# Amandaynzhou/CGC-Net

Measured on AMD Instinct MI355X. Metric: cell-graphs/sec (fwd+bwd), batch=32, ~1800 nodes/16 feat, higher is better.
Workload: dtype f32; 1 GPU; C3: full CGC-Net (3 conv blocks + 2 DiffPool) fwd+bwd+Adam, 32 graphs/GPU/step, ~1803 nodes, ~16159 edges/graph, 16 feat, max_num_nodes=11404 (C1=1140, C2=114), flags=shipped; global_batch=32, nodes_per_batch=57711, parallelism=dp1, includes=CSR build + fwd + loss + bwd + grad all-reduce + Adam, step_sequencer=True, node_order=draw order, fused_adam=True, optimiser=cgc_adam_step (one launch; torch fused Adam arithmetic)

## Files before the change

cgc-net_amd/_abi.py:

```python
import ctypes as C

P, I, F, D, L = C.c_void_p, C.c_int, C.c_float, C.c_double, C.c_int64

ABI_VERSION = 28

PROTOTYPES = {
    'cgc_abi_version': [],
    'cgc_csr_bad_edges_offset': [L, I, I],
    'cgc_csr_build': [P, L, I, I, P, P, P, P, P, P, P, P],
    'cgc_collate': [P, I, I, P, P, P, I, P, P, L, P, P],
    'cgc_farthest_point_sample': [P, P, I, I, P, P, P, P],
    'cgc_farthest_point_sample_table16': [P, P, I, I, P, P, P, P],
    'cgc_radius_knn_ws_ints': [I, I],
    'cgc_radius_knn': [P, P, I, I, F, I, I, P, P, P, P, P],
    'cgc_knn_emit_edges': [P, P, I, I, L, P, P],
    'cgc_nuclei_lds_max_pixels': [],
    'cgc_nuclei_ws_bytes': [I],
    'cgc_nuclei_label_pass': [P, I, I, I, I, P, P, P, P],
    'cgc_nuclei_big_ws_bytes': [I, L],
    'cgc_nuclei_features': [P, P, I, I, I, I, P, P, I, I, L, P, P, P, P, P],
    'cgc_bgr_to_gray': [P, L, P, P],
    'cgc_label_ws_bytes': [I, I, I],
    'cgc_label_components': [P, I, I, I, I, I, I, P, P, P, P],
    'cgc_label_sizes': [P, I, I, I, P, P],
# ... 74 lines not shown
    'cgc_region_outline_count': [P, P, I, I, I, I, I, P, P, P, P],
    'cgc_region_outline_cracks': [P, P, I, I, I, I, I, P, P, L, P, P, P],
    'cgc_region_outline_loops': [L, P, P, P, P, P],
    'cgc_region_outline_keys': [L, L, P, P, P, P, P, P],
    'cgc_region_outline_tables': [L, L, P, P, P, P, P, P, P, P, P],
    'cgc_region_outline_scatter': [L, L, I, P, P, P, P, P, P, P, P, P, P],
    'cgc_region_outline_compact': [L, L, P, P, P, P, P],
    'cgc_edge_renorm': [P, P, I, F, P, P],
    'cgc_csr_transpose_vals': [P, P, P, I, P, P],
    'cgc_csr_invdeg': [P, P, I, P, P],
    'cgc_graph_build': [P, L, I, F, P, P, P, P, P, P, P, P, P, P, P],
    'cgc_graph_build_local': [P, L, I, P, P, I, I, I, F, P, P, P, P, P, P, P, P, P, P, P],
    'cgc_graph_local_max_nodes': [],
    'cgc_spmm': [P, P, P, P, P, P, P, P, I, I, P],
    'cgc_spmm_graphs': [P, P, P, P, P, P, P, P, I, I, I, P, I, I, I, P, P],
    'cgc_gemm_f32': [I, I, I, I, I, F, P, I, P, I, F, P, I, P, I, L, L, L, P, I, I, I, P, P, P, P, P, P, P, P, L, I, P],
    'cgc_gemm_ws_floats': [],
    'cgc_gemm_split_count': [],
    'cgc_gemm_half_count': [],
    'cgc_gemm_half_ws_floats': [],
    'cgc_gemm_half_min_work': [L],
    'cgc_gemm_tuning': [I],
    'cgc_reduce_batch_sum': [P, P, I, L, F, P],
    'cgc_reduce_batched': [P, P, I, I, I, F, P],
    'cgc_stats_blocks': [I, I],
    'cgc_stats_ws_floats': [I, I],
    'cgc_l2norm_act_stats': [P, I, I, I, I, P, P, P, P, P],
    'cgc_bn_finalize': [P, I, D, F, F, P, P, P, P, P],
    'cgc_l2norm_act_bn': [P, I, I, I, I, P, P, P, D, F, F, P, P, P, P, P, P],
    'cgc_sage_wide_fwd': [P, I, P, P, I, I, I, I, I, P, I, P, I, P, D, F, F, P, P, P, P, P, P],
    'cgc_bn_running_stats': [P, P, I, F, P, P, P],
    'cgc_bn_act_apply': [P, I, I, I, P, P, P, P, P, I, P, I, P],
    'cgc_bn_bwd_reduce': [P, I, P, I, I, I, P, P, P, P, P],
    'cgc_bn_act_l2_bwd': [P, I, P, P, I, I, I, I, I, P, P, P, P, D, P, P, P, P],
    'cgc_sage_narrow_fwd': [P, I, P, P, I, I, I, I, I, P, P, I, P, D, F, F, P, P, P, P, P, P],
    'cgc_sage_narrow_ws_floats': [I, I, I],
    'cgc_sage_narrow_bwd': [P, I, P, P, I, I, I, I, I, P, P, P, P, D, P, I, I, P, P, I, P, P, P],
    'cgc_colsum': [P, I, I, I, P, P, P],
    'cgc_softmax_fwd': [P, I, I, I, P, P],
    'cgc_softmax_bwd': [P, P, I, I, I, P, P, P, P],
    'cgc_segment_max_fwd': [P, P, I, I, I, P, P, P],
    'cgc_segment_max_bwd': [P, P, I, I, P, P],
    'cgc_segment_max_bwd_full': [P, P, P, I, I, I, P, P],
    'cgc_jk_supported': [I],
    'cgc_jk_matrix_core': [I],
    'cgc_jk_lstm_fwd': [P, I, I, I, P, P, P, P, P, P, P],
    'cgc_jk_lstm_bwd': [P, P, I, I, I, P, P, P, P, P, P, P, P, P, P],
    'cgc_jk_bwd_ws_floats': [I],
    'cgc_jk_lstm_bwd_params': [P, P, I, I, I, P, P, P, P, P, P, P, P, P],
    'cgc_jk_lstm_bwd_flat': [P, P, I, I, I, P, P, P, P, P, P, P, P, P],
    'cgc_jk_param_grad_floats': [I],
    'cgc_jk_unpack_param_grads': [P, I, P, P],
# ... 46 lines not shown
```

cgc-net_amd/csrc/exec.hip:

```cpp
#include <stdio.h>
#include <stdlib.h>
#include <string.h>

#include "common.hpp"
#include "groups.hpp"

struct CatArgs {
  const float* src[4];
  int ld[4], width[4], off[4];
};
__global__ __launch_bounds__(256) void k_cat_cols(float* __restrict__ dst, int ldd, long long rows, int total_w, CatArgs a, int nsrc,
                                                  int accumulate) {
  const long long total = rows * total_w;
  for (long long i = blockIdx.x * 256ll + threadIdx.x; i < total; i += (long long)gridDim.x * 256) {
    const long long r = i / total_w;
    const int c = (int)(i - r * total_w);
    int s = 0;
#pragma unroll
    for (int k = 1; k < 4; ++k)
      if (k < nsrc && c >= a.off[k]) s = k;
    const float v = a.src[s][r * a.ld[s] + (c - a.off[s])];
    float* p = dst + r * ldd + c;
    *p = accumulate ? *p + v : v;
  }
// ... 56 lines not shown
    off += n;
    if (off > high) high = off;
    return p;
  }
  int* i(size_t n) { return reinterpret_cast<int*>(f(n)); }
  size_t mark() const { return off; }
  void release(size_t m) { off = m; }
};

struct Ctx {
  cgc_stream_t s;
  bool dry;
  Arena* scratch;
  float* gws;
  int64_t gws_floats;
  int gemm_mode = CGC_GEMM_EXACT;
};

static int fail_at(int rc, const char* what, int line) {
  static const bool verbose = getenv("CGC_EXEC_DEBUG") != nullptr;
  if (verbose) fprintf(stderr, "cgc exec.hip:%d: rc %d from %s\n", line, rc, what);
  return rc;
}
#define CALL(expr)                                              \
  do {                                                          \
    if (!c.dry) {                                               \
      const int rc__ = (expr);                                  \
      if (rc__ != 0) return fail_at(rc__, #expr, __LINE__);     \
    }                                                           \
  } while (0)
// ... 149 lines not shown
  if (!fused) {
    TRY(gemm(c, 0, 0, n, F, fin, agg, lda, p.W, F, 0.f, s.hn, F, p.b));
    if (batch_stats)
      CALL(cgc_l2norm_act_bn(s.hn, n, F, 1, d.act, s.hn, s.rinv, ws, d.count, p.eps, p.mom, p.rm, p.rv, p.nbt, s.mean, s.istd, c.s));
    else
      CALL(cgc_l2norm_act_stats(s.hn, n, F, 1, d.act, s.hn, s.rinv, nullptr, nullptr, c.s));
  }
  if (d.has_bn && d.eval) CALL(cgc_bn_running_stats(p.rm, p.rv, F, p.eps, s.mean, s.istd, c.s));
  CALL(cgc_bn_act_apply(s.hn, n, F, d.act, d.has_bn ? s.mean : nullptr, s.istd, p.gamma, p.beta, y, ldy, y2, ldy2, c.s));
  c.scratch->release(m);
  return 0;
}

int layer_bwd(const Ctx& c, const cgc_level_desc& d, const LayerP& p, const LayerS& s, const float* agg, int lda, int n, int fin, int F,
              const float* dy, int ldy, float* dagg, int ldd, float* dwdb, float* sums) {
  const size_t m = c.scratch->mark();
  const int mode = d.has_bn ? 2 : 0;
  const size_t slot_floats = (size_t)(cgc_stats_blocks(n, F) > 1 ? cgc_stats_blocks(n, F) : 1) * 2 * F;
  if (d.has_bn) {
    float* ws = c.scratch->f(slot_floats);
    CALL(cgc_bn_bwd_reduce(dy, ldy, s.hn, n, F, d.act, s.mean, s.istd, sums, ws, c.s));
  }
  float* db = d.has_bias ? dwdb + (size_t)fin * F : nullptr;
  if (F <= 32 && fin <= 32) {
    float* ws = c.scratch->f((size_t)cgc_sage_narrow_ws_floats(n, fin, F));
    CALL(cgc_sage_narrow_bwd(dy, ldy, s.hn, s.rinv, n, F, d.act, 1, mode, s.mean, s.istd, p.gamma, d.has_bn ? sums : nullptr, d.count, agg,
                             lda, fin, p.W, dagg, ldd, dwdb, ws, c.s));
  } else {
    float* dh = c.scratch->f((size_t)n * F);
    float* ws = db ? c.scratch->f(slot_floats) : nullptr;
    CALL(cgc_bn_act_l2_bwd(dy, ldy, s.hn, s.rinv, n, F, d.act, 1, mode, s.mean, s.istd, p.gamma, d.has_bn ? sums : nullptr, d.count, dh, db, ws,
                           c.s));
    if (dagg) TRY(gemm(c, 0, 1, n, fin, F, dh, F, p.W, F, 0.f, dagg, ldd));
    TRY(gemm_tn_rows(c, agg, lda, fin, dh, F, F, n, dwdb));
  }
  c.scratch->release(m);
  return 0;
}

inline bool pairable(int fin_e, int F_e, int fin_p, int F_p) { return fin_e == fin_p && F_e == F_p && fin_e <= 32 && F_e <= 32; }

int layer_fwd_pair(const Ctx& c, const cgc_level_desc& d, const LayerP* p, const LayerS* s, const float* const* agg, int lda, int n, int fin, int F,
// ... 7 lines not shown
    float* ws = batch_stats ? c.scratch->f(stats_ws_floats(n, F)) : nullptr;
    g[i] = SnFwdPtrs{agg[i], p[i].W, p[i].b, s[i].hn, s[i].rinv, ws};
    bn[i] = SnFwdBn{p[i].eps, p[i].mom, p[i].rm, p[i].rv, p[i].nbt, s[i].mean, s[i].istd};
    ap[i] = BnApplyPtrs{s[i].hn, d.has_bn ? s[i].mean : nullptr, s[i].istd, p[i].gamma, p[i].beta, y[i], y2[i], ldy2[i]};
  }
  CALL(sage_narrow_fwd_groups(g, bn, 2, lda, n, fin, F, 1, d.act, batch_stats, d.count, as_stream(c.s)));
  if (d.has_bn && d.eval)
    for (int i = 0; i < 2; ++i) CALL(cgc_bn_running_stats(p[i].rm, p[i].rv, F, p[i].eps, s[i].mean, s[i].istd, c.s));
  CALL(bn_act_apply_groups(ap, 2, n, F, d.act, ldy, as_stream(c.s)));
  c.scratch->release(m);
  return 0;
}

int layer_bwd_pair(const Ctx& c, const cgc_level_desc& d, const LayerP* p, const LayerS* s, const float* const* agg, int lda, int n, int fin, int F,
                   const float* const* dy, int ldy, float* const* dagg, int ldd, float* const* dwdb, float* const* sums) {
  const size_t m = c.scratch->mark();
  const int mode = d.has_bn ? 2 : 0;
  const size_t slot_floats = (size_t)(cgc_stats_blocks(n, F) > 1 ? cgc_stats_blocks(n, F) : 1) * 2 * F;
  if (d.has_bn) {
    BnRedPtrs r[2];
    for (int i = 0; i < 2; ++i) r[i] = BnRedPtrs{dy[i], s[i].hn, s[i].mean, s[i].istd, c.scratch->f(slot_floats)};
    CALL(bn_bwd_reduce_groups(r, sums, 2, ldy, n, F, d.act, as_stream(c.s)));
  }
  SnBwdPtrs g[2];
  for (int i = 0; i < 2; ++i)
    g[i] = SnBwdPtrs{dy[i], s[i].hn, s[i].rinv, s[i].mean, s[i].istd, p[i].gamma, d.has_bn ? sums[i] : nullptr, agg[i], p[i].W, dagg[i],
                     c.scratch->f((size_t)cgc_sage_narrow_ws_floats(n, fin, F))};
  CALL(sage_narrow_bwd_groups(g, dwdb, 2, ldy, n, F, d.act, 1, mode, d.count, lda, fin, ldd, as_stream(c.s)));
  c.scratch->release(m);
  return 0;
}

struct Level {
  const cgc_level_desc& d;
  int n, B, R, fin, H, E, AH, C, D, D3, wp, wt, ldp, ldC, ldP, ldW, ftot, npad_jk, seg_nmax;
  bool dense, pool, tall;
  float *At, *An, *invd, *ge1, *agg0, *pair[2], *xcat, *aggk[2], *hp3, *cat_e, *HS, *CS, *jk_out, *x12, *S, *P;
  float *G, *keep;
  bool reg;
  double reg_numel, reg_rows;
  int* arg;
  LayerS L[6];
  cgc_level_grad_layout gl;
// ... 109 lines not shown

int aggregate(const Ctx& c, const Level& L, const cgc_graph* g, const int* gptr, const float* h, int ldh, int w, float* out) {
  if (!L.dense) {
    CALL(cgc_spmm_graphs(g->rowptr, g->col, nullptr, g->val, nullptr, g->inv_d, h, out, L.n, w, w, gptr, L.B, L.d.nmax, 0, nullptr, c.s));
    return 0;
  }
  return bgemm(c, T3{L.An, L.B, L.R, L.R, L.R}, T3{const_cast<float*>(h), L.B, L.R, w, ldh}, T3{out, L.B, L.R, w, w}, 0, 0);
}
int aggregate_t(const Ctx& c, const Level& L, const cgc_graph* g, const int* gptr, const float* dy, int ldy, int w, float* dx) {
  if (!L.dense) {
    CALL(cgc_spmm_graphs(g->t_rowptr, g->t_col, nullptr, g->t_val, g->inv_d, nullptr, dy, dx, L.n, w, w, gptr, L.B, L.d.nmax, 0, nullptr, c.s));
    return 0;
  }
  return bgemm(c, T3{L.An, L.B, L.R, L.R, L.R}, T3{const_cast<float*>(dy), L.B, L.R, w, ldy}, T3{dx, L.B, L.R, w, w}, 1, 0);
}

int reg_fwd(const Ctx& c, Level& L, const cgc_graph* g, const int* gptr, const float* A_in, const float* A_out, float* reg_out) {
  const cgc_level_desc& d = L.d;
  const int C = L.C, B = L.B;
  if (!L.dense) {
    TRY(gemm(c, 1, 0, C, C, 0, L.S, L.ldC, L.S, L.ldC, 0.f, L.G, C, nullptr, B, 0, 0, (int64_t)C * C, gptr, 2, d.nmax));
  } else {
    const T3 s3{L.S, B, L.R, C, L.ldC};
    TRY(bgemm(c, s3, s3, T3{L.G, B, C, C, C}, 1, 0));
  }
  const size_t m = c.scratch->mark();
  float* ws = c.scratch->f((size_t)cgc_diffpool_reg_ws_floats());
  if (L.dense)
    CALL(cgc_diffpool_reg_fwd(L.S, L.n, C, L.ldC, L.G, A_out, B, d.renorm ? L.At : A_in, (int64_t)L.n * L.R, nullptr, L.reg_numel, L.reg_rows,
                              ws, reg_out, reg_out + 1, L.keep, c.s));
// ... 94 lines not shown
  if (d.jk) {
    d_cat = sc.f((size_t)n * D3);
    const size_t m = sc.mark();
    float* ws = sc.f((size_t)cgc_jk_bwd_ws_floats(H));
    CALL(cgc_jk_lstm_bwd_flat(L.cat_e, d_embed, n, L.npad_jk, H, jk->lstm, jk->w_att, jk->b_att, L.HS, L.CS, d_cat, grads + L.gl.jk, ws, c.s));
    sc.release(m);
  }
  float* dagg[2];
  const int ldg = L.ldp;
  float* const gcat = dagg1 != nullptr ? dagg1 : sc.f((size_t)n * ldg);
  dagg[1] = gcat;
  TRY(layer_bwd(c, d, layer_params(d, emb, 2, 2), L.L[2], L.aggk[1], wp, n, H, L.E, d_cat + 2 * H, D3, dagg[1], ldg, grads + L.gl.W[2], sums(2)));
  float* dpair = nullptr;
  for (int k = 1; k >= 0; --k) {
    dpair = sc.f((size_t)n * wp);
    TRY(aggregate_t(c, L, g, gptr, dagg[k], ldg, wp, dpair));
    if (L.pool) TRY(cat2(c, dpair, wp, n, d_cat + k * H, D3, H, dx12 + k * AH, 2 * AH, AH, 1));
    else TRY(add1(c, dpair, wp, n, d_cat + k * H, D3, H));
    const bool first = k == 0;
    const bool need_in = !first || L.dense;
    const float* ain = first ? L.agg0 : L.aggk[k - 1];
    const int lda = first ? fin : wp;
    const int fi_e = L.width_in(k), fi_p = L.width_in(3 + k);
    float *de = nullptr, *dp = nullptr;
    int ldd = ldg;
    if (need_in && !first) {
      de = dagg[0] = L.dense ? gcat + wp : sc.f((size_t)n * wp);
      dp = de + H;
    } else if (need_in) {
      de = gcat + 2 * wp;
      dp = L.pool ? sc.f((size_t)n * ldg) : nullptr;
    }
    if (L.pool && pairable(fi_e, H, fi_p, AH)) {
// ... 6 lines not shown
      float* sm[2] = {sums(k), sums(3 + k)};
      TRY(layer_bwd_pair(c, d, pp, ss, ag, lda, n, fi_e, H, dyy, wp, dg, ldd, dw, sm));
    } else {
      TRY(layer_bwd(c, d, layer_params(d, emb, k, k), L.L[k], ain, lda, n, fi_e, H, dpair, wp, de, ldd, grads + L.gl.W[k], sums(k)));
      if (L.pool)
        TRY(layer_bwd(c, d, layer_params(d, pl, k, 3 + k), L.L[3 + k], first ? ain : ain + H, lda, n, fi_p, AH, dpair + H, wp, dp, ldd,
                      grads + L.gl.W[3 + k], sums(3 + k)));
    }
    if (first && L.dense) {
      if (L.pool) TRY(add1(c, de, ldg, n, dp, ldg, fin));
      TRY(aggregate_t(c, L, g, gptr, de, ldg, fin, d_x_in));
      float* dAn = sc.f((size_t)n * R);
      TRY(bgemm(c, T3{gcat, B, R, L.wt, L.wt}, T3{L.xcat, B, R, L.wt, L.wt}, T3{dAn, B, R, R, R}, 0, 1));
      CALL(cgc_adj_prep_bwd(A_in, L.An, L.invd, L.ge1, dAn, gAt, n, R, d.renorm ? d.renorm_p : -1.f, d_A_in, c.s));
    }
  }
  return 0;
}

int level_bwd(const Ctx& c, Level& L, const cgc_block_params* emb, const cgc_block_params* pl, const cgc_jk_params* jk, const cgc_graph* g,
              const int* gptr, const float* x_in, const float* A_in, const float* d_readout, const float* d_xo, const float* d_ao, float* grads,
              float* d_x_in, float* d_A_in, const float* d_reg = nullptr) {
  const cgc_level_desc& d = L.d;
  Arena& sc = *c.scratch;
  const int n = L.n, H = L.H, AH = L.AH, wp = L.wp, C = L.C, D = L.D, B = L.B, R = L.R;
  float* d_embed = sc.f((size_t)n * D);
  CALL(cgc_segment_max_bwd_full(d_readout, L.arg, gptr, B, D, L.seg_nmax, d_embed, c.s));
  float *dx12 = nullptr, *gAt = nullptr;
  if (L.pool) {
    float *Gs = nullptr, *coef = nullptr;
// ... 56 lines not shown
                  grads + L.gl.W[5] + (int64_t)AH * C + C));
    return level_bwd_blocks(c, L, emb, pl, jk, g, gptr, x_in, A_in, d_embed, dx12, dagg1, gAt, grads, d_x_in, d_A_in);
  }
  return level_bwd_blocks(c, L, emb, pl, jk, g, gptr, x_in, A_in, d_embed, nullptr, nullptr, nullptr, grads, d_x_in, d_A_in);
}

template <class Body>
int run_level(const cgc_level_desc* d, float* saved, float* scratch, cgc_stream_t stream, Body&& body) {
  Level L(*d);
  Arena sv(saved), sc(scratch);
  L.layout_saved(sv);
  L.layout_grads();
  Ctx c{stream, false, &sc, nullptr, cgc_gemm_ws_floats()};
  c.gws = sc.f((size_t)c.gws_floats);
  c.gemm_mode = (d->flags & 2) ? CGC_GEMM_SPLIT_BF16 : (d->flags & 4) ? CGC_GEMM_SPLIT_F16 : CGC_GEMM_EXACT;
  return body(c, L);
}

}

extern "C" int cgc_level_supported(const cgc_level_desc* d) {
  if (d == nullptr || d->level < 1 || d->level > 3 || d->B < 1 || d->B > 65535 || d->n < 1) return 0;
  if (d->fin < 1 || d->H < 1 || d->E < 1 || d->act < 0 || d->act > 3) return 0;
  if (d->level >= 2 && (d->rows_per_graph < 1 || (long long)d->B * d->rows_per_graph != d->n)) return 0;
  if (d->level == 1 && (d->nmax < 1 || d->npad < d->nmax)) return 0;
  if (d->C > 0 && (d->AH < 1 || d->H + d->AH > 256 || (2 * d->AH) % 4 != 0)) return 0;
  if (d->C == 0 && d->level == 1) return 0;
  if ((d->flags & ~14) || (d->flags & 6) == 6) return 0;
  if ((d->flags & 8) && d->C == 0) return 0;
  if (d->jk && (d->E != d->H || !cgc_jk_matrix_core(d->H))) return 0;
// ... 71 lines not shown
```

cgc-net_amd/csrc/groups.hpp:

```cpp
#pragma once
#include "common.hpp"

struct SnFwdPtrs {
  const float *agg, *W, *bias;
  float *hn, *rinv, *ws;
};
struct SnFwdBn {
  float eps, momentum;
  float *running_mean, *running_var;
  int64_t* nbt;
  float *mean, *istd;
};
struct SnBwdPtrs {
  const float *dy, *hn, *rinv, *mean, *istd, *gamma, *sums, *agg, *W;
  float *dagg, *ws;
};
struct StatsFinPtrs {
  const float* ws;
  float *running_mean, *running_var, *mean, *istd;
  long long* nbt;
  float eps, momentum;
};
struct BnApplyPtrs {
  const float *hn, *mean, *istd, *gamma, *beta;
  float *y, *y2;
  int ldy2;
};
struct BnRedPtrs {
  const float *dy, *hn, *mean, *istd;
  float* ws;
};

int sage_narrow_fwd_groups(const SnFwdPtrs* g, const SnFwdBn* bn, int ng, int lda, int n, int K, int F, int normalize, int act, int stats,
                           double count, hipStream_t st);
int sage_narrow_bwd_groups(const SnBwdPtrs* g, float* const* dwdb, int ng, int ldy, int n, int F, int act, int normalize, int mode, double count,
                           int lda, int fin, int ldd, hipStream_t st);
int bn_act_apply_groups(const BnApplyPtrs* g, int ng, int n, int F, int act, int ldy, hipStream_t stream);
int bn_bwd_reduce_groups(const BnRedPtrs* g, float* const* sums, int ng, int ldy, int n, int F, int act, hipStream_t stream);
int launch_stats_finalize_groups(const StatsFinPtrs* g, int ng, int slots, int F, double count, hipStream_t stream);
int launch_stats_finalize(const float* ws, int slots, int F, double count, float eps, float momentum, float* running_mean,
                          float* running_var, float* mean, float* istd, int64_t* nbt, hipStream_t stream);
template <typename OUT, typename IN>
int launch_reduce_slots(const IN* ws0, OUT* out0, const IN* ws1, OUT* out1, int ng, int slots, int width, hipStream_t stream);
int reduce_batch_sum_rows(const float* ws, float* out, int parts, int rows, int width, int ldo, float beta, hipStream_t stream);
```

cgc-net_amd/csrc/rowops.hip:

```cpp
#include <type_traits>

#include "common.hpp"
#include "groups.hpp"

#define L2_EPS 1e-12f
#define RENORM_EPS 1e-15f
#define MAX_SLOTS 1024

template <int VEC, int MAXJ, int NQ>
__device__ __forceinline__ void col_reduce_store(float (&acc)[NQ][MAXJ][VEC], int F, int lpr, float* smem, float* slot) {
  const int lane = threadIdx.x & 63, wave = threadIdx.x >> 6;
#pragma unroll
  for (int q = 0; q < NQ; ++q)
#pragma unroll
    for (int j = 0; j < MAXJ; ++j)
#pragma unroll
      for (int v = 0; v < VEC; ++v)
        for (int o = 32; o >= lpr; o >>= 1) acc[q][j][v] += __shfl_xor(acc[q][j][v], o);
  if (wave > 0 && lane < lpr) {
#pragma unroll
    for (int q = 0; q < NQ; ++q)
#pragma unroll
      for (int j = 0; j < MAXJ; ++j)
#pragma unroll
// ... 84 lines not shown
  const int cl = threadIdx.x & 31, grp = threadIdx.x >> 5;
  const int c = blockIdx.x * 32 + cl;
  double s = 0.0;
  if (c < width) s = slot_col_sum(ws, c, slots, width);
  part[grp][cl] = s;
  __syncthreads();
  if (grp == 0 && c < width) out[c] = (OUT)slot_part_fold(part, cl);
}
template <typename OUT, typename IN>
int launch_reduce_slots(const IN* ws0, OUT* out0, const IN* ws1, OUT* out1, int ng, int slots, int width, hipStream_t stream) {
  hipLaunchKernelGGL((k_reduce_slots<OUT, IN>), dim3(ceil_div(width, 32), ng), dim3(32 * RS_GROUPS), 0, stream, ws0, out0, ws1, out1, slots, width);
  CGC_RETURN_IF_LAUNCH_FAILED();
  return 0;
}
template int launch_reduce_slots<float, float>(const float*, float*, const float*, float*, int, int, int, hipStream_t);

struct ColCfg {
  int vec, maxj, lpr, blocks;
  bool ok;
};
static ColCfg col_cfg(int n, int F, bool vec_ok) {
  ColCfg c;
  c.vec = vec_ok ? 4 : 1;
  c.ok = true;
  int chunks = F / c.vec;
  if (chunks <= 64) {
    c.maxj = 1;
    c.lpr = pick_lpr(chunks);
  } else {
    c.lpr = 64;
// ... 1257 lines not shown
```

cgc-net_amd/csrc/sagenarrow.hip:

```cpp
#include "common.hpp"
#include "groups.hpp"

#define L2_EPS 1e-12f
typedef float floatx16 __attribute__((ext_vector_type(16)));

template <int CTRL>
__device__ __forceinline__ float dpp_step(float v) {
  return v + __builtin_bit_cast(float, __builtin_amdgcn_mov_dpp(__builtin_bit_cast(int, v), CTRL, 0xF, 0xF, true));
}
__device__ __forceinline__ float half_sum(float v) {
  v = dpp_step<0xB1>(v);
  v = dpp_step<0x4E>(v);
  v = dpp_step<0x141>(v);
  v = dpp_step<0x140>(v);
  return v + __shfl_xor(v, 16);
}

#define SN_LDT 33

template <int FS, int ACT>
__global__ __launch_bounds__(256) void k_sage_narrow_bwd(const SnBwdPtrs p0, const SnBwdPtrs p1, int ldy, int n, int F, int ,
                                                         int normalize, int mode, float inv_count, int lda, int fin, int ldd, int tiles) {
  const bool second = blockIdx.y != 0;
  const float* __restrict__ dy = second ? p1.dy : p0.dy;
// ... 105 lines not shown
    float d = (xch[(0 * 17 + 16) * 64 + lane] + xch[(1 * 17 + 16) * 64 + lane]) + (xch[(2 * 17 + 16) * 64 + lane] + xch[(3 * 17 + 16) * 64 + lane]);
    d += __shfl_xor(d, 32);
    if (fok && half == 0) slot[fin * F + f] = d;
  }
}

static int sn_grid(int n) {
  const int tiles = ceil_div(n, 32);
  int g = ceil_div(tiles, 4);
  return g < 1024 ? g : 1024;
}

extern "C" int64_t cgc_sage_narrow_ws_floats(int n, int fin, int F) { return (int64_t)sn_grid(n > 0 ? n : 1) * (fin * F + F); }

int sage_narrow_bwd_groups(const SnBwdPtrs* g, float* const* dwdb, int ng, int ldy, int n, int F, int act, int normalize, int mode, double count,
                           int lda, int fin, int ldd, hipStream_t st) {
  if (F <= 0 || fin <= 0) return 0;
  if (F > 32 || fin > 32 || ng < 1 || ng > 2) return CGC_EINVAL;
  for (int i = 0; i < ng; ++i)
    if (g[i].ws == nullptr || dwdb[i] == nullptr || (g[i].dagg != nullptr && ldd < fin)) return CGC_EINVAL;
  const int width = fin * F + F;
  if (n <= 0) {
    for (int i = 0; i < ng; ++i) (void)hipMemsetAsync(dwdb[i], 0, sizeof(float) * width, st);
    return 0;
  }
  const int tiles = ceil_div(n, 32), grid = sn_grid(n);
  const float inv_count = (float)(1.0 / count);
  const int fs = (F + 1) / 2;
  const SnBwdPtrs& g1 = g[ng - 1];
  auto launch = [&](auto fs_c) {
    with_act(act, [&](auto act_c) {
      hipLaunchKernelGGL((k_sage_narrow_bwd<decltype(fs_c)::value, decltype(act_c)::value>), dim3(grid, ng), dim3(256), 0, st, g[0], g1, ldy, n,
                         F, act, normalize, mode, inv_count, lda, fin, ldd, tiles);
    });
  };
  if (fs <= 8) launch(std::integral_constant<int, 8>());
  else if (fs <= 10) launch(std::integral_constant<int, 10>());
  else launch(std::integral_constant<int, 16>());
  CGC_RETURN_IF_LAUNCH_FAILED();
  return launch_reduce_slots<float, float>(g[0].ws, dwdb[0], g1.ws, dwdb[ng - 1], ng, grid, width, st);
}

extern "C" int cgc_sage_narrow_bwd(const float* dy, int ldy, const float* hn, const float* rinv, int n, int F, int act, int normalize,
                                   int mode, const float* mean, const float* istd, const float* gamma, const float* sums, double count,
                                   const float* agg, int lda, int fin, const float* W, float* dagg, int ldd, float* dwdb, float* ws,
                                   cgc_stream_t stream_) {
  const SnBwdPtrs g{dy, hn, rinv, mean, istd, gamma, sums, agg, W, dagg, ws};
  float* const out[1] = {dwdb};
  return sage_narrow_bwd_groups(&g, out, 1, ldy, n, F, act, normalize, mode, count, lda, fin, ldd, as_stream(stream_));
}

template <int KS, int ACT>
__global__ __launch_bounds__(256) void k_sage_narrow_fwd(const SnFwdPtrs p0, const SnFwdPtrs p1, int lda, int n, int K, int F, int normalize,
                                                         int , int tiles) {
// ... 137 lines not shown
```

cgc-net_amd/csrc/spmm.hip:

```cpp
#include "common.hpp"

constexpr int GATHER_U = 9;

template <int VEC>
__global__ __launch_bounds__(256) void k_spmm(const int* __restrict__ rowptr, const int* __restrict__ col, const int* __restrict__ perm,
                                              const float* __restrict__ val, const float* __restrict__ pre,
                                              const float* __restrict__ post, const float* __restrict__ x, float* __restrict__ out,
                                              int n, int W, int ld, int lpr, int n_ctiles, int rows_per_block, int blocks_per_ct,
                                              int n_chunks, int nt_store, const int* __restrict__ gptr) {
  const int nb = gridDim.x, b = blockIdx.x;
  const int vb = (nb % 8 == 0) ? (b % 8) * (nb / 8) + b / 8 : b;
  const int per_chunk = blocks_per_ct * n_ctiles;
  const int chunk = vb / per_chunk;
  if (chunk >= n_chunks) return;
  const int rem = vb - chunk * per_chunk;
  const int ct = rem / blocks_per_ct, rb = rem - ct * blocks_per_ct;
  int row0, row_end;
  if (gptr != nullptr) {
    const int g0 = gptr[chunk], g1 = gptr[chunk + 1];
    row0 = g0 + rb * rows_per_block;
    if (row0 >= g1) return;
    row_end = min(row0 + rows_per_block, g1);
  } else {
    row0 = (chunk * blocks_per_ct + rb) * rows_per_block;
// ... 37 lines not shown
          } else {
            ww[u] = 0.f;
#pragma unroll
            for (int v = 0; v < VEC; ++v) xv[u].v[v] = 0.f;
          }
        }
#pragma unroll
        for (int u = 0; u < GATHER_U; ++u)
#pragma unroll
          for (int v = 0; v < VEC; ++v) acc[v] = fmaf(ww[u], xv[u].v[v], acc[v]);
      }
    }
    if (valid && colok) {
      const float ps = post != nullptr ? post[r] : 1.f;
      float* op = out + (size_t)r * ld + c0;
      if (nt_store && VEC == 4) {
        typedef float f4v __attribute__((ext_vector_type(4)));
        f4v o4 = {acc[0] * ps, acc[VEC > 1 ? 1 : 0] * ps, acc[VEC > 2 ? 2 : 0] * ps, acc[VEC > 3 ? 3 : 0] * ps};
        __builtin_nontemporal_store(o4, reinterpret_cast<f4v*>(op));
      } else {
        Vec<VEC> o;
#pragma unroll
        for (int v = 0; v < VEC; ++v) o.v[v] = acc[v] * ps;
        o.store(op);
      }
    }
  }
}

typedef float wide_f4 __attribute__((ext_vector_type(4)));

template <int CNT, bool VAL, bool PERM, bool PRE>
__device__ __forceinline__ void wide_batch(const int* __restrict__ col, const int* __restrict__ perm,
                                           const float* __restrict__ val, const float* __restrict__ pre,
                                           const float* __restrict__ xl, int W, int k, wide_f4& acc) {
  int cc[CNT];
  wide_f4 xv[CNT];
  float ww[CNT];
// ... 79 lines not shown
    const int e = rowptr[r + 1];
    f4v acc = {0.f, 0.f, 0.f, 0.f};
    int k = s;
    for (; k + U <= e; k += U) wide_batch<U, VAL, PERM, PRE>(col, perm, val, pre, xl, ld, k, acc);
    wide_tail<U - 1, VAL, PERM, PRE>(e - k, col, perm, val, pre, xl, ld, k, acc);
    if (post != nullptr) acc *= post[r];
    __builtin_nontemporal_store(acc, reinterpret_cast<f4v*>(out + (size_t)r * ld + c0));
    s = e;
  }
}

constexpr int SPMM_PASSES = 2, SPMM_CHUNK = 2048, SPMM_RUN = 2;

static int launch_gather(const int* rowptr, const int* col, const int* perm, const float* val, const float* pre, const float* post,
                         const float* x, float* out, int n, int width, int ld, const int* gptr, int B, int nmax, int order,
                         hipStream_t stream, const int* gorder = nullptr) {
  const bool vec = (width % 4 == 0) && (ld % 4 == 0) && aligned16(x) && aligned16(out);
  const int chunks = vec ? width / 4 : width;
  const int lpr = pick_lpr(chunks);
  const int n_ctiles = ceil_div(chunks, lpr);
  const int rpw = 64 / lpr;
  const int rows_per_block = 4 * rpw * SPMM_PASSES;
  int blocks_per_ct, n_chunks;
  if (gptr != nullptr && n_ctiles > 1) {
    blocks_per_ct = ceil_div(nmax, rows_per_block);
    n_chunks = B;
  } else {
    gptr = nullptr;
    const int chunk_rows = ceil_div(SPMM_CHUNK, rows_per_block) * rows_per_block;
    blocks_per_ct = chunk_rows / rows_per_block;
    n_chunks = ceil_div(n, chunk_rows);
  }
  if (vec && lpr == 64) {
    const int rpb = 4 * SPMM_RUN;
    if (gptr != nullptr) {
      blocks_per_ct = ceil_div(nmax, rpb);
    } else {
      const int chunk_rows = ceil_div(SPMM_CHUNK, rpb) * rpb;
      blocks_per_ct = chunk_rows / rpb;
      n_chunks = ceil_div(n, chunk_rows);
    }
    const int nbw = ceil_div(n_chunks * blocks_per_ct * n_ctiles, 8) * 8;
#define WIDE_LAUNCH(V, P, Q)                                                                                              \
  hipLaunchKernelGGL((k_spmm_wide<GATHER_U, V, P, Q>), dim3(nbw), dim3(CGC_BLOCK), 0, stream, rowptr, col, perm, val, pre, \
                     post, x, out, n, width, ld, n_ctiles, SPMM_RUN, blocks_per_ct, n_chunks, gptr, order, gorder)
    const bool hv = val != nullptr, hp = hv && perm != nullptr, hq = pre != nullptr;
    if (!hv && !hq) WIDE_LAUNCH(false, false, false);
    else if (!hv) WIDE_LAUNCH(false, false, true);
    else if (!hp && !hq) WIDE_LAUNCH(true, false, false);
    else if (!hp) WIDE_LAUNCH(true, false, true);
    else if (!hq) WIDE_LAUNCH(true, true, false);
    else WIDE_LAUNCH(true, true, true);
#undef WIDE_LAUNCH
    CGC_RETURN_IF_LAUNCH_FAILED();
    return 0;
  }
  int nb = n_chunks * blocks_per_ct * n_ctiles;
  nb = ceil_div(nb, 8) * 8;
  dim3 grid(nb), block(CGC_BLOCK);
  const int nt = n_ctiles > 1 ? 1 : 0;
  if (vec)
    hipLaunchKernelGGL(k_spmm<4>, grid, block, 0, stream, rowptr, col, perm, val, pre, post, x, out, n, width, ld, lpr,
                       n_ctiles, rows_per_block, blocks_per_ct, n_chunks, nt, gptr);
  else
    hipLaunchKernelGGL(k_spmm<1>, grid, block, 0, stream, rowptr, col, perm, val, pre, post, x, out, n, width, ld, lpr,
                       n_ctiles, rows_per_block, blocks_per_ct, n_chunks, nt, gptr);
  CGC_RETURN_IF_LAUNCH_FAILED();
  return 0;
}

extern "C" int cgc_spmm(const int* rowptr, const int* col, const int* perm, const float* val, const float* pre, const float* post,
                        const float* x, float* out, int n, int width, cgc_stream_t stream) {
  if (n <= 0 || width <= 0) return 0;
  return launch_gather(rowptr, col, perm, val, pre, post, x, out, n, width, width, nullptr, 0, 0, 0, as_stream(stream));
}

extern "C" int cgc_spmm_graphs(const int* rowptr, const int* col, const int* perm, const float* val, const float* pre,
                               const float* post, const float* x, float* out, int n, int width, int ld, const int* gptr, int B,
                               int nmax, int visit, const int* gorder, cgc_stream_t stream) {
  if (n <= 0 || width <= 0) return 0;
  if (ld < width) return CGC_EINVAL;
  const int trec = width > 64 ? cgc_timing_begin(CGC_TAG_SPMM_WIDE, n, width, ld, val != nullptr, 0, 0, 0, as_stream(stream)) : -1;
  const int rc = launch_gather(rowptr, col, perm, val, pre, post, x, out, n, width, ld, gptr, B, nmax, visit & 3, as_stream(stream), gorder);
  cgc_timing_end(trec, as_stream(stream));
  return rc;
}
```

include/cgc_hip.h:

```cpp
#ifndef CGC_HIP_H
#define CGC_HIP_H
#include <stdint.h>

#ifdef __cplusplus
extern "C" {
#endif

typedef void* cgc_stream_t;

#define CGC_EINVAL (-1)

#define CGC_ACT_IDENTITY 0
#define CGC_ACT_RELU 1
#define CGC_ACT_ELU 2
#define CGC_ACT_LEAKYRELU 3

#define CGC_ABI_VERSION 28
int cgc_abi_version(void);

int64_t cgc_csr_bad_edges_offset(int64_t E, int n, int add_diag);
int cgc_csr_build(const int64_t* edge_index, int64_t E, int n, int add_diag,
                  int* rowptr, int* col, int* rowidx, int* t_rowptr, int* t_col, int* t_perm,
                  int* ws, cgc_stream_t stream);

int cgc_collate(float* x, int n, int F, const float* mean, const float* stdv, const int* gptr, int B, int64_t* batch,
                int64_t* edge_index, int64_t E, const int* eptr, cgc_stream_t stream);

int cgc_farthest_point_sample(const float* pos, const int* gptr, int B, int max_nodes, const int* start, const int* optr,
                              int* out, cgc_stream_t stream);
int cgc_farthest_point_sample_table16(const float* pos, const int* gptr, int B, int max_nodes, const int* start,
                                      const int* optr, int* out, cgc_stream_t stream);

// ... 174 lines not shown
int cgc_csr_invdeg(const int* rowptr, const float* val, int n, float* out, cgc_stream_t stream);

int cgc_graph_build(const int64_t* edge_index, int64_t E, int n, float renorm_p, int* rowptr, int* col, int* rowidx, int* t_rowptr,
                    int* t_col, int* t_perm, float* val, float* t_val, float* inv_d, int* ws, cgc_stream_t stream);
int cgc_graph_local_max_nodes(void);
int cgc_graph_build_local(const int64_t* edge_index, int64_t E, int n, const int* gptr, const int* eptr, int B, int nmax, int emax,
                          float renorm_p, int* rowptr, int* col, int* rowidx, int* t_rowptr, int* t_col, int* t_perm, float* val,
                          float* t_val, float* inv_d, int* ws, cgc_stream_t stream);

int cgc_spmm(const int* rowptr, const int* col, const int* perm, const float* val, const float* pre,
             const float* post, const float* x, float* out, int n, int width, cgc_stream_t stream);

int cgc_spmm_graphs(const int* rowptr, const int* col, const int* perm, const float* val, const float* pre,
                    const float* post, const float* x, float* out, int n, int width, int ld , const int* gptr, int B, int nmax, int visit, const int* gorder,
                    cgc_stream_t stream);

#define CGC_GEMM_EXACT 0
#define CGC_GEMM_SPLIT_BF16 1
#define CGC_GEMM_SPLIT_F16 2
int cgc_gemm_f32(int transA, int transB, int M, int N, int K, float alpha, const float* A, int lda,
                 const float* B, int ldb, float beta, float* C, int ldc, const float* bias, int batch,
                 int64_t strideA, int64_t strideB, int64_t strideC, const int* gptr, int ragged, int max_ragged,
                 int nx, const float* const* xA, const int* xlda, const int64_t* xstrideA,
                 const float* const* xB, const int* xldb, const int64_t* xstrideB, const int* xK,
                 float* ws, int64_t ws_floats, int mode, cgc_stream_t stream);
int64_t cgc_gemm_split_count(void);
int64_t cgc_gemm_half_count(void);
int64_t cgc_gemm_half_ws_floats(void);
int64_t cgc_gemm_half_min_work(int64_t v);
int64_t cgc_gemm_ws_floats(void);
// ... 52 lines not shown
int cgc_sage_wide_fwd(const float* agg, int lda, const float* W, const float* bias, int n, int K, int F, int normalize, int act,
                      float* hn, int ldh, float* rinv, int stats, float* ws, double count, float eps, float momentum,
                      float* running_mean, float* running_var, int64_t* num_batches_tracked, float* mean, float* istd,
                      cgc_stream_t stream);

int cgc_sage_narrow_fwd(const float* agg, int lda, const float* W, const float* bias, int n, int K, int F, int normalize, int act,
                        float* hn, float* rinv, int stats, float* ws, double count, float eps, float momentum,
                        float* running_mean, float* running_var, int64_t* num_batches_tracked, float* mean, float* istd,
                        cgc_stream_t stream);

int64_t cgc_sage_narrow_ws_floats(int n, int fin, int F);
int cgc_sage_narrow_bwd(const float* dy, int ldy, const float* hn, const float* rinv, int n, int F, int act, int normalize,
                        int mode, const float* mean, const float* istd, const float* gamma, const float* sums, double count,
                        const float* agg, int lda, int fin, const float* W, float* dagg, int ldd, float* dwdb, float* ws,
                        cgc_stream_t stream);

int cgc_dense_rownorm_fwd(const float* A, int R, int C, float* out, float* invd, float* ge1, cgc_stream_t stream);
int cgc_dense_rownorm_bwd(const float* dOut, const float* Anorm, const float* invd, const float* ge1, int R, int C,
                          float* dA, cgc_stream_t stream);
int cgc_dense_renorm_fwd(const float* A, int R, int C, float p, float* out, cgc_stream_t stream);
int cgc_dense_renorm_bwd(const float* A, const float* dOut, int R, int C, float p, float* dA, cgc_stream_t stream);

int cgc_adj_prep_fwd(const float* A, int R, int C, float p, float* At, float* An, float* invd, float* ge1, cgc_stream_t stream);
int cgc_adj_prep_bwd(const float* A, const float* An, const float* invd, const float* ge1, const float* gAn, const float* gAt,
                     int R, int C, float p, float* dA, cgc_stream_t stream);

int cgc_cat_cols(float* dst, int ldd, int rows, int nsrc, const float* const* srcs, const int* lds, const int* widths,
                 int accumulate, cgc_stream_t stream);
int cgc_transpose(const float* src, int lds, int rows, int cols, float* dst, int ldd, cgc_stream_t stream);

// ... 107 lines not shown
```

Measured before the change: 2859 graphs/s.

## Fuse residual add into transposed SpMM and batch deferred slot reductions

In the sparse-level backward, the transposed aggregation now adds the concat/pool gradient contributions directly in the SpMM epilogue, so the separate cat2/add1 elementwise launches go away. The narrow SAGE backward can also defer its per-slot weight-gradient fold into a list, and all folds for a level run at the end in one multi-entry kernel launch. This cuts launch count and an extra pass over the gradient buffers. In exchange, scratch workspaces are now allocated before the mark so they outlive their layer until the deferred fold runs, which raises peak scratch use. The fold list is capped at eight entries and returns an error if it overflows.

```diff
diff --git a/cgc-net_amd/_abi.py b/cgc-net_amd/_abi.py
--- a/cgc-net_amd/_abi.py
+++ b/cgc-net_amd/_abi.py
@@ -2,7 +2,7 @@
 
 P, I, F, D, L = C.c_void_p, C.c_int, C.c_float, C.c_double, C.c_int64
 
-ABI_VERSION = 28
+ABI_VERSION = 29
 
 PROTOTYPES = {
     'cgc_abi_version': [],
@@ -112,6 +112,7 @@
     'cgc_graph_local_max_nodes': [],
     'cgc_spmm': [P, P, P, P, P, P, P, P, I, I, P],
     'cgc_spmm_graphs': [P, P, P, P, P, P, P, P, I, I, I, P, I, I, I, P, P],
+    'cgc_spmm_graphs_add': [P, P, P, P, P, P, P, P, I, I, I, P, I, I, I, P, I, P, P, P, P],
     'cgc_gemm_f32': [I, I, I, I, I, F, P, I, P, I, F, P, I, P, I, L, L, L, P, I, I, I, P, P, P, P, P, P, P, P, L, I, P],
     'cgc_gemm_ws_floats': [],
     'cgc_gemm_split_count': [],
@@ -134,6 +135,7 @@
     'cgc_sage_narrow_fwd': [P, I, P, P, I, I, I, I, I, P, P, I, P, D, F, F, P, P, P, P, P, P],
     'cgc_sage_narrow_ws_floats': [I, I, I],
     'cgc_sage_narrow_bwd': [P, I, P, P, I, I, I, I, I, P, P, P, P, D, P, I, I, P, P, I, P, P, P],
+    'cgc_reduce_slots_list': [I, P, P, P, P, P],
     'cgc_colsum': [P, I, I, I, P, P, P],
     'cgc_softmax_fwd': [P, I, I, I, P, P],
     'cgc_softmax_bwd': [P, P, I, I, I, P, P, P, P],
diff --git a/cgc-net_amd/csrc/exec.hip b/cgc-net_amd/csrc/exec.hip
--- a/cgc-net_amd/csrc/exec.hip
+++ b/cgc-net_amd/csrc/exec.hip
@@ -94,6 +94,7 @@
   Arena* scratch;
   float* gws;
   int64_t gws_floats;
+  SlotFoldList* folds = nullptr;
   int gemm_mode = CGC_GEMM_EXACT;
 };
 
@@ -273,6 +274,8 @@
 
 int layer_bwd(const Ctx& c, const cgc_level_desc& d, const LayerP& p, const LayerS& s, const float* agg, int lda, int n, int fin, int F,
               const float* dy, int ldy, float* dagg, int ldd, float* dwdb, float* sums) {
+  const bool narrow = F <= 32 && fin <= 32;
+  float* const nws = narrow ? c.scratch->f((size_t)cgc_sage_narrow_ws_floats(n, fin, F)) : nullptr;
   const size_t m = c.scratch->mark();
   const int mode = d.has_bn ? 2 : 0;
   const size_t slot_floats = (size_t)(cgc_stats_blocks(n, F) > 1 ? cgc_stats_blocks(n, F) : 1) * 2 * F;
@@ -281,10 +284,10 @@
     CALL(cgc_bn_bwd_reduce(dy, ldy, s.hn, n, F, d.act, s.mean, s.istd, sums, ws, c.s));
   }
   float* db = d.has_bias ? dwdb + (size_t)fin * F : nullptr;
-  if (F <= 32 && fin <= 32) {
-    float* ws = c.scratch->f((size_t)cgc_sage_narrow_ws_floats(n, fin, F));
-    CALL(cgc_sage_narrow_bwd(dy, ldy, s.hn, s.rinv, n, F, d.act, 1, mode, s.mean, s.istd, p.gamma, d.has_bn ? sums : nullptr, d.count, agg,
-                             lda, fin, p.W, dagg, ldd, dwdb, ws, c.s));
+  if (narrow) {
+    const SnBwdPtrs g{dy, s.hn, s.rinv, s.mean, s.istd, p.gamma, d.has_bn ? sums : nullptr, agg, p.W, dagg, nws};
+    float* const out[1] = {dwdb};
+    CALL(sage_narrow_bwd_groups(&g, out, 1, ldy, n, F, d.act, 1, mode, d.count, lda, fin, ldd, as_stream(c.s), c.folds));
   } else {
     float* dh = c.scratch->f((size_t)n * F);
     float* ws = db ? c.scratch->f(slot_floats) : nullptr;
@@ -322,6 +325,8 @@
 
 int layer_bwd_pair(const Ctx& c, const cgc_level_desc& d, const LayerP* p, const LayerS* s, const float* const* agg, int lda, int n, int fin, int F,
                    const float* const* dy, int ldy, float* const* dagg, int ldd, float* const* dwdb, float* const* sums) {
+  float* nws[2];
+  for (int i = 0; i < 2; ++i) nws[i] = c.scratch->f((size_t)cgc_sage_narrow_ws_floats(n, fin, F));
   const size_t m = c.scratch->mark();
   const int mode = d.has_bn ? 2 : 0;
   const size_t slot_floats = (size_t)(cgc_stats_blocks(n, F) > 1 ? cgc_stats_blocks(n, F) : 1) * 2 * F;
@@ -332,9 +337,8 @@
   }
   SnBwdPtrs g[2];
   for (int i = 0; i < 2; ++i)
-    g[i] = SnBwdPtrs{dy[i], s[i].hn, s[i].rinv, s[i].mean, s[i].istd, p[i].gamma, d.has_bn ? sums[i] : nullptr, agg[i], p[i].W, dagg[i],
-                     c.scratch->f((size_t)cgc_sage_narrow_ws_floats(n, fin, F))};
-  CALL(sage_narrow_bwd_groups(g, dwdb, 2, ldy, n, F, d.act, 1, mode, d.count, lda, fin, ldd, as_stream(c.s)));
+    g[i] = SnBwdPtrs{dy[i], s[i].hn, s[i].rinv, s[i].mean, s[i].istd, p[i].gamma, d.has_bn ? sums[i] : nullptr, agg[i], p[i].W, dagg[i], nws[i]};
+  CALL(sage_narrow_bwd_groups(g, dwdb, 2, ldy, n, F, d.act, 1, mode, d.count, lda, fin, ldd, as_stream(c.s), c.folds));
   c.scratch->release(m);
   return 0;
 }
@@ -474,6 +478,14 @@
   }
   return bgemm(c, T3{L.An, L.B, L.R, L.R, L.R}, T3{const_cast<float*>(dy), L.B, L.R, w, ldy}, T3{dx, L.B, L.R, w, w}, 1, 0);
 }
+int aggregate_t_add(const Ctx& c, const Level& L, const cgc_graph* g, const int* gptr, const float* dy, int w, float* dx, const float* a, int lda,
+                    int wa, const float* b, int ldb, int wb) {
+  const float* s[2] = {a, b};
+  const int l[2] = {lda, ldb}, wd[2] = {wa, wb};
+  CALL(cgc_spmm_graphs_add(g->t_rowptr, g->t_col, nullptr, g->t_val, g->inv_d, nullptr, dy, dx, L.n, w, w, gptr, L.B, L.d.nmax, 0, nullptr,
+                           b != nullptr ? 2 : 1, s, l, wd, c.s));
+  return 0;
+}
 
 int reg_fwd(const Ctx& c, Level& L, const cgc_graph* g, const int* gptr, const float* A_in, const float* A_out, float* reg_out) {
   const cgc_level_desc& d = L.d;
@@ -598,9 +610,13 @@
   float* dpair = nullptr;
   for (int k = 1; k >= 0; --k) {
     dpair = sc.f((size_t)n * wp);
-    TRY(aggregate_t(c, L, g, gptr, dagg[k], ldg, wp, dpair));
-    if (L.pool) TRY(cat2(c, dpair, wp, n, d_cat + k * H, D3, H, dx12 + k * AH, 2 * AH, AH, 1));
-    else TRY(add1(c, dpair, wp, n, d_cat + k * H, D3, H));
+    if (!L.dense) {
+      TRY(aggregate_t_add(c, L, g, gptr, dagg[k], wp, dpair, d_cat + k * H, D3, H, L.pool ? dx12 + k * AH : nullptr, 2 * AH, AH));
+    } else {
+      TRY(aggregate_t(c, L, g, gptr, dagg[k], ldg, wp, dpair));
+      if (L.pool) TRY(cat2(c, dpair, wp, n, d_cat + k * H, D3, H, dx12 + k * AH, 2 * AH, AH, 1));
+      else TRY(add1(c, dpair, wp, n, d_cat + k * H, D3, H));
+    }
     const bool first = k == 0;
     const bool need_in = !first || L.dense;
     const float* ain = first ? L.agg0 : L.aggk[k - 1];
@@ -637,6 +653,10 @@
       TRY(bgemm(c, T3{gcat, B, R, L.wt, L.wt}, T3{L.xcat, B, R, L.wt, L.wt}, T3{dAn, B, R, R, R}, 0, 1));
       CALL(cgc_adj_prep_bwd(A_in, L.An, L.invd, L.ge1, dAn, gAt, n, R, d.renorm ? d.renorm_p : -1.f, d_A_in, c.s));
     }
+  }
+  if (c.folds != nullptr) {
+    CALL(launch_reduce_slots_list(*c.folds, as_stream(c.s)));
+    c.folds->n = 0;
   }
   return 0;
 }
@@ -723,6 +743,8 @@
   Ctx c{stream, false, &sc, nullptr, cgc_gemm_ws_floats()};
   c.gws = sc.f((size_t)c.gws_floats);
   c.gemm_mode = (d->flags & 2) ? CGC_GEMM_SPLIT_BF16 : (d->flags & 4) ? CGC_GEMM_SPLIT_F16 : CGC_GEMM_EXACT;
+  SlotFoldList folds;
+  c.folds = &folds;
   return body(c, L);
 }
 
diff --git a/cgc-net_amd/csrc/groups.hpp b/cgc-net_amd/csrc/groups.hpp
--- a/cgc-net_amd/csrc/groups.hpp
+++ b/cgc-net_amd/csrc/groups.hpp
@@ -31,10 +31,22 @@
   float* ws;
 };
 
+struct SlotFold {
+  const float* ws;
+  float* out;
+  int slots, width;
+};
+constexpr int SLOT_FOLD_MAX = 8;
+struct SlotFoldList {
+  SlotFold e[SLOT_FOLD_MAX];
+  int n = 0;
+};
+int launch_reduce_slots_list(const SlotFoldList& l, hipStream_t stream);
+
 int sage_narrow_fwd_groups(const SnFwdPtrs* g, const SnFwdBn* bn, int ng, int lda, int n, int K, int F, int normalize, int act, int stats,
                            double count, hipStream_t st);
 int sage_narrow_bwd_groups(const SnBwdPtrs* g, float* const* dwdb, int ng, int ldy, int n, int F, int act, int normalize, int mode, double count,
-                           int lda, int fin, int ldd, hipStream_t st);
+                           int lda, int fin, int ldd, hipStream_t st, SlotFoldList* defer = nullptr);
 int bn_act_apply_groups(const BnApplyPtrs* g, int ng, int n, int F, int act, int ldy, hipStream_t stream);
 int bn_bwd_reduce_groups(const BnRedPtrs* g, float* const* sums, int ng, int ldy, int n, int F, int act, hipStream_t stream);
 int launch_stats_finalize_groups(const StatsFinPtrs* g, int ng, int slots, int F, double count, hipStream_t stream);
diff --git a/cgc-net_amd/csrc/rowops.hip b/cgc-net_amd/csrc/rowops.hip
--- a/cgc-net_amd/csrc/rowops.hip
+++ b/cgc-net_amd/csrc/rowops.hip
@@ -122,6 +122,46 @@
   return 0;
 }
 template int launch_reduce_slots<float, float>(const float*, float*, const float*, float*, int, int, int, hipStream_t);
+
+__global__ __launch_bounds__(32 * RS_GROUPS) void k_reduce_slots_list(const SlotFoldList l) {
+  SlotFold e = l.e[0];
+#pragma unroll
+  for (int i = 1; i < SLOT_FOLD_MAX; ++i)
+    if ((int)blockIdx.y == i) e = l.e[i];
+  const float* __restrict__ ws = e.ws;
+  float* __restrict__ out = e.out;
+  const int slots = e.slots, width = e.width;
+  if ((int)blockIdx.x * 32 >= width) return;
+  __shared__ double part[RS_GROUPS][32];
+  const int cl = threadIdx.x & 31, grp = threadIdx.x >> 5;
+  const int c = blockIdx.x * 32 + cl;
+  double s = 0.0;
+  if (c < width) s = slot_col_sum(ws, c, slots, width);
+  part[grp][cl] = s;
+  __syncthreads();
+  if (grp == 0 && c < width) out[c] = (float)slot_part_fold(part, cl);
+}
+int launch_reduce_slots_list(const SlotFoldList& l, hipStream_t stream) {
+  if (l.n <= 0) return 0;
+  if (l.n > SLOT_FOLD_MAX) return CGC_EINVAL;
+  int wmax = 0;
+  for (int i = 0; i < l.n; ++i) {
+    if (l.e[i].ws == nullptr || l.e[i].out == nullptr || l.e[i].slots < 0 || l.e[i].width <= 0) return CGC_EINVAL;
+    if (l.e[i].width > wmax) wmax = l.e[i].width;
+  }
+  hipLaunchKernelGGL(k_reduce_slots_list, dim3(ceil_div(wmax, 32), l.n), dim3(32 * RS_GROUPS), 0, stream, l);
+  CGC_RETURN_IF_LAUNCH_FAILED();
+  return 0;
+}
+extern "C" int cgc_reduce_slots_list(int count, const float* const* ws, float* const* out, const int* slots, const int* widths,
+                                     cgc_stream_t stream) {
+  if (count < 0 || count > SLOT_FOLD_MAX) return CGC_EINVAL;
+  if (count == 0) return 0;
+  if (ws == nullptr || out == nullptr || slots == nullptr || widths == nullptr) return CGC_EINVAL;
+  SlotFoldList l;
+  for (int i = 0; i < count; ++i) l.e[l.n++] = SlotFold{ws[i], out[i], slots[i], widths[i]};
+  return launch_reduce_slots_list(l, as_stream(stream));
+}
 
 struct ColCfg {
   int vec, maxj, lpr, blocks;
diff --git a/cgc-net_amd/csrc/sagenarrow.hip b/cgc-net_amd/csrc/sagenarrow.hip
--- a/cgc-net_amd/csrc/sagenarrow.hip
+++ b/cgc-net_amd/csrc/sagenarrow.hip
@@ -143,11 +143,12 @@
 extern "C" int64_t cgc_sage_narrow_ws_floats(int n, int fin, int F) { return (int64_t)sn_grid(n > 0 ? n : 1) * (fin * F + F); }
 
 int sage_narrow_bwd_groups(const SnBwdPtrs* g, float* const* dwdb, int ng, int ldy, int n, int F, int act, int normalize, int mode, double count,
-                           int lda, int fin, int ldd, hipStream_t st) {
+                           int lda, int fin, int ldd, hipStream_t st, SlotFoldList* defer) {
   if (F <= 0 || fin <= 0) return 0;
   if (F > 32 || fin > 32 || ng < 1 || ng > 2) return CGC_EINVAL;
   for (int i = 0; i < ng; ++i)
     if (g[i].ws == nullptr || dwdb[i] == nullptr || (g[i].dagg != nullptr && ldd < fin)) return CGC_EINVAL;
+  if (defer != nullptr && defer->n + ng > SLOT_FOLD_MAX) return CGC_EINVAL;
   const int width = fin * F + F;
   if (n <= 0) {
     for (int i = 0; i < ng; ++i) (void)hipMemsetAsync(dwdb[i], 0, sizeof(float) * width, st);
@@ -167,6 +168,10 @@
   else if (fs <= 10) launch(std::integral_constant<int, 10>());
   else launch(std::integral_constant<int, 16>());
   CGC_RETURN_IF_LAUNCH_FAILED();
+  if (defer != nullptr) {
+    for (int i = 0; i < ng; ++i) defer->e[defer->n++] = SlotFold{g[i].ws, dwdb[i], grid, width};
+    return 0;
+  }
   return launch_reduce_slots<float, float>(g[0].ws, dwdb[0], g1.ws, dwdb[ng - 1], ng, grid, width, st);
 }
 
diff --git a/cgc-net_amd/csrc/spmm.hip b/cgc-net_amd/csrc/spmm.hip
--- a/cgc-net_amd/csrc/spmm.hip
+++ b/cgc-net_amd/csrc/spmm.hip
@@ -1,13 +1,20 @@
 #include "common.hpp"
 
 constexpr int GATHER_U = 9;
+
+struct SpmmAddend {
+  const float* src[2];
+  int ld[2];
+  int off1;
+  int nsrc;
+};
 
 template <int VEC>
 __global__ __launch_bounds__(256) void k_spmm(const int* __restrict__ rowptr, const int* __restrict__ col, const int* __restrict__ perm,
                                               const float* __restrict__ val, const float* __restrict__ pre,
                                               const float* __restrict__ post, const float* __restrict__ x, float* __restrict__ out,
                                               int n, int W, int ld, int lpr, int n_ctiles, int rows_per_block, int blocks_per_ct,
-                                              int n_chunks, int nt_store, const int* __restrict__ gptr) {
+                                              int n_chunks, int nt_store, const int* __restrict__ gptr, const SpmmAddend add) {
   const int nb = gridDim.x, b = blockIdx.x;
   const int vb = (nb % 8 == 0) ? (b % 8) * (nb / 8) + b / 8 : b;
   const int per_chunk = blocks_per_ct * n_ctiles;
@@ -75,14 +82,22 @@
     if (valid && colok) {
       const float ps = post != nullptr ? post[r] : 1.f;
       float* op = out + (size_t)r * ld + c0;
+      Vec<VEC> o;
+#pragma unroll
+      for (int v = 0; v < VEC; ++v) o.v[v] = acc[v] * ps;
+      if (add.nsrc > 0) {
+#pragma unroll
+        for (int v = 0; v < VEC; ++v) {
+          const int c = c0 + v;
+          const int s = (add.nsrc > 1 && c >= add.off1) ? 1 : 0;
+          o.v[v] += add.src[s][(size_t)r * add.ld[s] + (c - (s ? add.off1 : 0))];
+        }
+      }
       if (nt_store && VEC == 4) {
         typedef float f4v __attribute__((ext_vector_type(4)));
-        f4v o4 = {acc[0] * ps, acc[VEC > 1 ? 1 : 0] * ps, acc[VEC > 2 ? 2 : 0] * ps, acc[VEC > 3 ? 3 : 0] * ps};
+        f4v o4 = {o.v[0], o.v[VEC > 1 ? 1 : 0], o.v[VEC > 2 ? 2 : 0], o.v[VEC > 3 ? 3 : 0]};
         __builtin_nontemporal_store(o4, reinterpret_cast<f4v*>(op));
       } else {
-        Vec<VEC> o;
-#pragma unroll
-        for (int v = 0; v < VEC; ++v) o.v[v] = acc[v] * ps;
         o.store(op);
       }
     }
@@ -192,7 +207,11 @@
 
 static int launch_gather(const int* rowptr, const int* col, const int* perm, const float* val, const float* pre, const float* post,
                          const float* x, float* out, int n, int width, int ld, const int* gptr, int B, int nmax, int order,
-                         hipStream_t stream, const int* gorder = nullptr) {
+                         hipStream_t stream, const int* gorder = nullptr, const SpmmAddend* addend = nullptr) {
+  SpmmAddend add;
+  if (addend != nullptr) add = *addend;
+  else add = SpmmAddend{{nullptr, nullptr}, {0, 0}, 0, 0};
+  if (add.nsrc > 0 && post != nullptr) return CGC_EINVAL;
   const bool vec = (width % 4 == 0) && (ld % 4 == 0) && aligned16(x) && aligned16(out);
   const int chunks = vec ? width / 4 : width;
   const int lpr = pick_lpr(chunks);
@@ -210,6 +229,7 @@
     n_chunks = ceil_div(n, chunk_rows);
   }
   if (vec && lpr == 64) {
+    if (add.nsrc > 0) return CGC_EINVAL;
     const int rpb = 4 * SPMM_RUN;
     if (gptr != nullptr) {
       blocks_per_ct = ceil_div(nmax, rpb);
@@ -239,10 +259,10 @@
   const int nt = n_ctiles > 1 ? 1 : 0;
   if (vec)
     hipLaunchKernelGGL(k_spmm<4>, grid, block, 0, stream, rowptr, col, perm, val, pre, post, x, out, n, width, ld, lpr,
-                       n_ctiles, rows_per_block, blocks_per_ct, n_chunks, nt, gptr);
+                       n_ctiles, rows_per_block, blocks_per_ct, n_chunks, nt, gptr, add);
   else
     hipLaunchKernelGGL(k_spmm<1>, grid, block, 0, stream, rowptr, col, perm, val, pre, post, x, out, n, width, ld, lpr,
-                       n_ctiles, rows_per_block, blocks_per_ct, n_chunks, nt, gptr);
+                       n_ctiles, rows_per_block, blocks_per_ct, n_chunks, nt, gptr, add);
   CGC_RETURN_IF_LAUNCH_FAILED();
   return 0;
 }
@@ -253,13 +273,35 @@
   return launch_gather(rowptr, col, perm, val, pre, post, x, out, n, width, width, nullptr, 0, 0, 0, as_stream(stream));
 }
 
+extern "C" int cgc_spmm_graphs_add(const int* rowptr, const int* col, const int* perm, const float* val, const float* pre,
+                                   const float* post, const float* x, float* out, int n, int width, int ld, const int* gptr, int B,
+                                   int nmax, int visit, const int* gorder, int nadd, const float* const* add_src,
+                                   const int* add_ld, const int* add_width, cgc_stream_t stream) {
+  if (n <= 0 || width <= 0) return 0;
+  if (ld < width) return CGC_EINVAL;
+  if (nadd < 0 || nadd > 2) return CGC_EINVAL;
+  SpmmAddend add{{nullptr, nullptr}, {0, 0}, 0, nadd};
+  if (nadd > 0) {
+    if (add_src == nullptr || add_ld == nullptr || add_width == nullptr) return CGC_EINVAL;
+    int total = 0;
+    for (int i = 0; i < nadd; ++i) {
+      if (add_src[i] == nullptr || add_width[i] <= 0 || add_ld[i] < add_width[i]) return CGC_EINVAL;
+      add.src[i] = add_src[i];
+      add.ld[i] = add_ld[i];
+      total += add_width[i];
+    }
+    if (total != width) return CGC_EINVAL;
+    add.off1 = add_width[0];
+  }
+  const int trec = width > 64 ? cgc_timing_begin(CGC_TAG_SPMM_WIDE, n, width, ld, val != nullptr, 0, 0, 0, as_stream(stream)) : -1;
+  const int rc = launch_gather(rowptr, col, perm, val, pre, post, x, out, n, width, ld, gptr, B, nmax, visit & 3, as_stream(stream), gorder, &add);
+  cgc_timing_end(trec, as_stream(stream));
+  return rc;
+}
+
 extern "C" int cgc_spmm_graphs(const int* rowptr, const int* col, const int* perm, const float* val, const float* pre,
                                const float* post, const float* x, float* out, int n, int width, int ld, const int* gptr, int B,
                                int nmax, int visit, const int* gorder, cgc_stream_t stream) {
-  if (n <= 0 || width <= 0) return 0;
-  if (ld < width) return CGC_EINVAL;
-  const int trec = width > 64 ? cgc_timing_begin(CGC_TAG_SPMM_WIDE, n, width, ld, val != nullptr, 0, 0, 0, as_stream(stream)) : -1;
-  const int rc = launch_gather(rowptr, col, perm, val, pre, post, x, out, n, width, ld, gptr, B, nmax, visit & 3, as_stream(stream), gorder);
-  cgc_timing_end(trec, as_stream(stream));
-  return rc;
-}
+  return cgc_spmm_graphs_add(rowptr, col, perm, val, pre, post, x, out, n, width, ld, gptr, B, nmax, visit, gorder, 0, nullptr, nullptr, nullptr,
+                             stream);
+}
diff --git a/include/cgc_hip.h b/include/cgc_hip.h
--- a/include/cgc_hip.h
+++ b/include/cgc_hip.h
@@ -15,7 +15,7 @@
 #define CGC_ACT_ELU 2
 #define CGC_ACT_LEAKYRELU 3
 
-#define CGC_ABI_VERSION 28
+#define CGC_ABI_VERSION 29
 int cgc_abi_version(void);
 
 int64_t cgc_csr_bad_edges_offset(int64_t E, int n, int add_diag);
@@ -220,6 +220,11 @@
 int cgc_spmm_graphs(const int* rowptr, const int* col, const int* perm, const float* val, const float* pre,
                     const float* post, const float* x, float* out, int n, int width, int ld , const int* gptr, int B, int nmax, int visit, const int* gorder,
                     cgc_stream_t stream);
+
+int cgc_spmm_graphs_add(const int* rowptr, const int* col, const int* perm, const float* val, const float* pre,
+                        const float* post, const float* x, float* out, int n, int width, int ld, const int* gptr, int B, int nmax,
+                        int visit, const int* gorder, int nadd, const float* const* add_src, const int* add_ld,
+                        const int* add_width, cgc_stream_t stream);
 
 #define CGC_GEMM_EXACT 0
 #define CGC_GEMM_SPLIT_BF16 1
@@ -302,6 +307,8 @@
                         int mode, const float* mean, const float* istd, const float* gamma, const float* sums, double count,
                         const float* agg, int lda, int fin, const float* W, float* dagg, int ldd, float* dwdb, float* ws,
                         cgc_stream_t stream);
+int cgc_reduce_slots_list(int count, const float* const* ws, float* const* out, const int* slots, const int* widths,
+                          cgc_stream_t stream);
 
 int cgc_dense_rownorm_fwd(const float* A, int R, int C, float* out, float* invd, float* ge1, cgc_stream_t stream);
 int cgc_dense_rownorm_bwd(const float* dOut, const float* Anorm, const float* invd, const float* ge1, int R, int C,
```

Result: no change. 2865 graphs/s, median of 6 (+0.2%).
